# DoHoonKim8/halo2-lasso

Measured on AMD Instinct MI355X. Metric: lasso_prove_time_ms, lower is better.
Workload: dtype u256 (BN254 Fr/Fq, 8x u32 Montgomery); 1 GPU; 2^24 AND Lasso lookup (32-bit operands, 4 chunks of 8+8 bits); lookups_per_proof=16777216, pcs=multilinear KZG (BN254), proof_bytes=64256, parallelism=1 GPU

## Files before the change

### bindings/rust/src/sys.rs

```rust
#![allow(non_camel_case_types, dead_code)]
use halo2_curves::bn256::{Fr, G1Affine, G2Affine};
use std::os::raw::{c_char, c_int, c_void};

pub type lh_status = c_int;
pub const LH_OK: lh_status = 0;
pub const LH_ERR_INVALID_SUMCHECK: lh_status = -1;
pub const LH_ERR_INVALID_PCS_PARAM: lh_status = -2;
pub const LH_ERR_INVALID_PCS_OPEN: lh_status = -3;
pub const LH_ERR_INVALID_SNARK: lh_status = -4;
pub const LH_ERR_SERIALIZATION: lh_status = -5;
pub const LH_ERR_TRANSCRIPT: lh_status = -6;
pub const LH_ERR_DEVICE: lh_status = -7;
pub const LH_ERR_ARG: lh_status = -8;

pub const LH_SC_MAX_TERMS: usize = 48;
pub const LH_SC_MAX_FACTORS: usize = 4;
pub const LH_SC_EVALUATIONS: c_int = 0;
pub const LH_SC_COEFFICIENTS: c_int = 1;
pub const LH_LASSO_MAX_CHUNKS: usize = 8;
pub const LH_LASSO_MAX_MEMORIES: usize = 16;
pub const LH_LASSO_MAX_TERMS: usize = 16;
pub const LH_RCCL_UNIQUE_ID_BYTES: usize = 128;

#[repr(C)] pub struct lh_ctx { _p: [u8; 0] }
// ... 112 lines not shown
    pub preprocess_comms: *const G1Affine,
    pub num_permutation_polys: usize,
    pub permutation_comms: *const G1Affine,
    pub num_lasso_lookups: usize,
    pub lasso_lookups: *const lh_hp_lasso_lookup,
}
#[repr(C)]
pub struct lh_hp_circuit {
    pub user: *mut c_void,
    pub synthesize: Option<unsafe extern "C" fn(*mut c_void, usize, *const Fr, usize, *mut *const c_void, usize) -> c_int>,
}

#[repr(C)]
#[derive(Clone, Copy, Debug, Default)]
pub struct lh_lasso_route {
    pub open_small_depth: u32,
    pub open_small_passes: u32,
    pub eq_factored_rounds: u32,
    pub standard_rounds: u32,
    pub rw_leaf_rounds: u32,
    pub resident_tails: u32,
    pub resident_rounds: u32,
    pub packed_ts_pairs: u32,
    pub derived_commitments: u32,
    pub sorted_dim_reuse: u32,
    pub sharded_rounds: u32,
    pub shard_exchanges: u32,
    pub window_table_jobs: u32,
    pub open_precommit: u32,
    pub resident_layers: u32,
    pub pp_folds: u32,
    pub msm_half_batches: u32,
    pub reserved: [u32; 7],
}

extern "C" {
    pub fn lh_last_error() -> *const c_char;
    pub fn lh_version() -> *const c_char;
    pub fn lh_ctx_create(device_id: c_int, out: *mut *mut lh_ctx) -> lh_status;
    pub fn lh_ctx_destroy(ctx: *mut lh_ctx);
    pub fn lh_ctx_sync(ctx: *mut lh_ctx) -> lh_status;
    pub fn lh_ctx_stream(ctx: *mut lh_ctx) -> *mut c_void;
    pub fn lh_alloc(ctx: *mut lh_ctx, bytes: usize, d_out: *mut *mut c_void) -> lh_status;
    pub fn lh_free(ctx: *mut lh_ctx, d_ptr: *mut c_void) -> lh_status;
    pub fn lh_upload(ctx: *mut lh_ctx, d_dst: *mut c_void, src: *const c_void, bytes: usize) -> lh_status;
    pub fn lh_download(ctx: *mut lh_ctx, dst: *mut c_void, d_src: *const c_void, bytes: usize) -> lh_status;
    pub fn lh_fr_from_u64(ctx: *mut lh_ctx, d_in: *const u64, n: usize, d_out: *mut Fr) -> lh_status;
    pub fn lh_fr_from_u32(ctx: *mut lh_ctx, d_in: *const u32, n: usize, d_out: *mut Fr) -> lh_status;
    pub fn lh_fr_batch_invert(ctx: *mut lh_ctx, d_in: *const Fr, n: usize, d_out: *mut Fr) -> lh_status;
    pub fn lh_fix_var(ctx: *mut lh_ctx, d_in: *const Fr, n_in: usize, x: *const Fr, d_out: *mut Fr) -> lh_status;
    pub fn lh_eq_xy(ctx: *mut lh_ctx, y: *const Fr, num_vars: usize, d_out: *mut Fr) -> lh_status;
    pub fn lh_evaluate(ctx: *mut lh_ctx, d_polys: *const *const Fr, num_polys: usize, num_vars: usize,
                       point: *const Fr, out_evals: *mut Fr) -> lh_status;
    pub fn lh_lincomb(ctx: *mut lh_ctx, d_polys: *const *const Fr, w: *const Fr, num_polys: usize, n: usize,
                      d_out: *mut Fr) -> lh_status;
    pub fn lh_sumcheck_prove(ctx: *mut lh_ctx, prover_kind: c_int, num_vars: usize, expr: *const lh_sop,
                             d_polys: *const *const Fr, num_polys: usize, ys: *const Fr, num_ys: usize,
                             sum: *const Fr, t: *mut lh_transcript, out_challenges: *mut Fr, out_evals: *mut Fr) -> lh_status;
    pub fn lh_sumcheck_prove_expr(ctx: *mut lh_ctx, num_vars: usize, expr: *const lh_expr, d_polys: *const *const Fr,
                                  num_polys: usize, challenges: *const Fr, num_challenges: usize, ys: *const Fr,
                                  num_ys: usize, sum: *const Fr, t: *mut lh_transcript, out_challenges: *mut Fr,
                                  out_evals: *mut Fr) -> lh_status;
    pub fn lh_sumcheck_verify(prover_kind: c_int, num_vars: usize, degree: usize, sum: *const Fr,
                              t: *mut lh_transcript, out_eval: *mut Fr, out_x: *mut Fr) -> lh_status;
    pub fn lh_gkr_fractional_prove(ctx: *mut lh_ctx, num_batching: usize, num_vars: usize,
                                   claimed_p_0s: *const *const Fr, claimed_q_0s: *const *const Fr,
// ... 68 lines not shown
```

### halo2-lasso_amd/__init__.py

```python
import ctypes as C

from . import _ffi
from ._ffi import (lh_fr, lh_g1, lh_sop, lh_evaluation, lh_lasso_table, lh_transcript,
                   LH_SC_EVALUATIONS, LH_SC_COEFFICIENTS)

R_MOD = 0x30644E72E131A029B85045B68181585D2833E84879B9709143E1F593F0000001
Q_MOD = 0x30644E72E131A029B85045B68181585D97816A916871CA8D3C208C16D87CFD47
_MONT = 1 << 256
_MONT_INV_R = pow(_MONT, -1, R_MOD)
_MONT_INV_Q = pow(_MONT, -1, Q_MOD)

SUBTABLE_IDENTITY, SUBTABLE_AND, SUBTABLE_XOR = 0, 1, 2


class Error(Exception):
    code = None


class InvalidSumcheck(Error):
    code = _ffi.LH_ERR_INVALID_SUMCHECK


class InvalidPcsParam(Error):
    code = _ffi.LH_ERR_INVALID_PCS_PARAM
# ... 857 lines not shown
    ctx._comm_keepalive = None


def shard_of(column, rank, size, shard_bit):
    rho = size.bit_length() - 1
    n = len(column)
    return column.reshape(n >> (shard_bit + rho), size, 1 << shard_bit)[:, rank, :].reshape(-1).copy()


def shard_poly(poly, rank, size, shard_bit):
    rho = size.bit_length() - 1
    n_local = (1 << poly.num_vars) >> rho
    out = poly.ctx.alloc(32 * n_local)
    _check(poly.ctx.lib.lh_shard_extract(poly.ctx.h, poly.ptr, n_local, shard_bit, rho, rank, 32, out.ptr))
    return MultilinearPolynomial(poly.ctx, out, poly.num_vars - rho)


def lasso_prove_sharded(pp, table, num_vars, dims_local, transcript):
    if len(dims_local) != table.c:
        raise ArgumentError("expected %d dim columns" % table.c)
    t = table.to_c()
    _check(pp.ctx.lib.lh_lasso_prove_sharded(pp.ctx.h, pp.h, C.byref(t), num_vars, _ptr_array(dims_local), transcript.p))


def lasso_last_timing(ctx):
    out = (C.c_double * _ffi.LH_LASSO_NUM_PHASES)()
    _check(ctx.lib.lh_lasso_last_timing(ctx.h, out))
    names = ["witness", "commit", "surge", "leaves", "gkr", "evals", "open_n", "open_l", "total"]
    return dict(zip(names, list(out)))


ROUTE_FIELDS = ["open_small_depth", "open_small_passes", "eq_factored_rounds", "standard_rounds", "rw_leaf_rounds",
                "resident_tails", "resident_rounds", "packed_ts_pairs", "derived_commitments", "sorted_dim_reuse",
                "sharded_rounds", "shard_exchanges", "window_table_jobs", "open_precommit", "resident_layers", "pp_folds", "msm_half_batches"]


def lasso_last_route(ctx):
    out = (C.c_uint32 * 24)()
    _check(ctx.lib.lh_lasso_last_route(ctx.h, out))
    return dict(zip(ROUTE_FIELDS, [int(v) for v in out]))


def set_option(ctx, name, value):
    _check(ctx.lib.lh_ctx_set_option(ctx.h, name.encode(), int(value)))


def get_option(ctx, name):
    out = C.c_int64(0)
    _check(ctx.lib.lh_ctx_get_option(ctx.h, name.encode(), C.byref(out)))
    return int(out.value)


def profile_enable(ctx, on=True):
    _check(ctx.lib.lh_profile_enable(ctx.h, int(on)))


def profile_read(ctx):
    n = C.c_size_t()
    _check(ctx.lib.lh_profile_read(ctx.h, None, 0, C.byref(n)))
    arr = (_ffi.lh_prof_rec * max(n.value, 1))()
    _check(ctx.lib.lh_profile_read(ctx.h, arr, n.value, C.byref(n)))
    return [dict(name=r.name.decode(), ms=r.ms, bytes=r.bytes, muls=r.muls, items=r.items) for r in arr[:n.value]]


from . import expression
```

### halo2-lasso_amd/csrc/dev.cpp

```cpp
#include <string.h>
#include <stdlib.h>
#include <ctype.h>
#include <sched.h>
#include <atomic>
#include <condition_variable>
#include <mutex>
#include <thread>
#include <functional>
#include <memory>
#include <emmintrin.h>
#include <hip/hip_ext.h>
#include <vector>
#include <chrono>
#include "dev.hpp"

namespace lh {

static thread_local std::string g_last_error;
void set_last_error(const char* msg) { g_last_error = msg ? msg : ""; }
const char* get_last_error() { return g_last_error.c_str(); }

Arena::~Arena() {
  for (auto& b : blocks_) (void)hipFree(b.p);
}
// ... 25 lines not shown
    if (want < bytes) want = bytes;
    void* p = nullptr;
    LH_HIP(hipMalloc(&p, want));
    blocks_.push_back(Block{(char*)p, want, 0});
    cur_ = blocks_.size() - 1;
  }
}

void Arena::release(Mark m) {
  if (blocks_.empty()) return;
  for (size_t i = m.block + 1; i < blocks_.size(); i++) blocks_[i].used = 0;
  cur_ = m.block;
  blocks_[cur_].used = m.used;
}

void Ctx::opt_in_lds(const void* fn, int bytes) {
  for (const void* f : lds_opted)
    if (f == fn) return;
  LH_HIP(hipFuncSetAttribute(fn, hipFuncAttributeMaxDynamicSharedMemorySize, bytes));
  lds_opted.push_back(fn);
}

static const struct {
  const char* name;
  int64_t Options::*field;
  int64_t lo, hi;
} OPTION_TABLE[] = {
    {"open_small_min_vars", &Options::open_small_min_vars, 0, 64}, {"open_small_depth", &Options::open_small_depth, 0, 2},
    {"sc_eq_factoring", &Options::sc_eq_factoring, 0, 1},          {"lasso_pack_ts", &Options::lasso_pack_ts, 0, 1},
    {"sc_tail", &Options::sc_tail, 0, 1},                          {"sc_tail_max_len", &Options::sc_tail_max_len, 0, (int64_t)1 << 20},
    {"shard_exchange_log", &Options::shard_exchange_log, 0, 40},   {"msm_window_tables", &Options::msm_window_tables, 0, 40},
    {"open_precommit", &Options::open_precommit, 0, 64},           {"gkr_resident", &Options::gkr_resident, 0, 1},
    {"sc_pp_fold", &Options::sc_pp_fold, 0, 2},                    {"msm_half_batches", &Options::msm_half_batches, 0, 1},
    {"comm_round", &Options::comm_round, 0, 2},
};

int64_t* Options::find(const char* name) {
  if (!name) return nullptr;
  for (const auto& o : OPTION_TABLE)
    if (strcmp(o.name, name) == 0) return &(this->*o.field);
  return nullptr;
}
bool Options::in_range(const char* name, int64_t value) {
  if (!name) return false;
  for (const auto& o : OPTION_TABLE)
    if (strcmp(o.name, name) == 0) return value >= o.lo && value <= o.hi;
  return false;
}

Options::Options() {
  for (const auto& o : OPTION_TABLE) {
    std::string env = "LH_";
    for (const char* p = o.name; *p; p++) env.push_back((char)toupper((unsigned char)*p));
    const char* e = getenv(env.c_str());
    if (!e || !*e) continue;
    const int64_t v = (int64_t)atoll(e);
    if (v < o.lo || v > o.hi) {
      fprintf(stderr, "[lasso-hip] %s=%s is outside [%lld, %lld]: ignored\n", env.c_str(), e, (long long)o.lo, (long long)o.hi);
      continue;
    }
    this->*o.field = v;
    if (o.field == &Options::open_small_min_vars) open_small_min_vars_forced = true;
  }
}

void Ctx::host_stamp(const char* tag) {
  if (!host_trace_on) return;
// ... 392 lines not shown
```

### halo2-lasso_amd/csrc/dev.hpp

```cpp
#pragma once
#include <hip/hip_runtime_api.h>
#include <stdint.h>
#include <stdarg.h>
#include <stdio.h>
#include <functional>
#include <string>
#include <vector>
#include <utility>
#include <stdexcept>

#include "../../include/lasso_hip.h"
#include "ec.cuh"

namespace lh {

struct Error : std::exception {
  int code;
  std::string msg;
  Error(int c, std::string m) : code(c), msg(std::move(m)) {}
  const char* what() const noexcept override { return msg.c_str(); }
};

void set_last_error(const char* msg);

// ... 50 lines not shown
  char name[40];
  double ms;
  double bytes;
  double muls;
  double items;
};

struct ScFinishArgs {
  uint32_t* ticket;
  uint32_t last_ticket;
  Fr* out_host;
  uint32_t* flag;
  uint32_t seq;
  uint64_t* wide;
  uint32_t tag;
  uint64_t* lanes;
};
constexpr uint32_t FIN_LANE_SUMS = 65536;
constexpr unsigned SC_LANE_TAG_SHIFT = 40;

struct Options {
  int64_t open_small_min_vars = 21;
  bool open_small_min_vars_forced = false;
  int64_t open_small_depth = 0;
  int64_t sc_eq_factoring = 1;
  int64_t lasso_pack_ts = 1;
  int64_t sc_tail = 1;
  int64_t sc_tail_max_len = 8192;
  int64_t shard_exchange_log = 19;
  int64_t open_precommit = 1;
  int64_t msm_window_tables = 0;
  int64_t sc_pp_fold = 1;
  int64_t msm_half_batches = 1;
  int64_t gkr_resident = 1;
  int64_t comm_round = 0;
  Options();
  int64_t* find(const char* name);
  static bool in_range(const char* name, int64_t value);
};
struct RouteStats {
  uint32_t v[LH_LASSO_ROUTE_WORDS] = {0};
  enum { OPEN_DEPTH, OPEN_PASSES, EF_ROUNDS, STD_ROUNDS, RW_ROUNDS, TAILS, TAIL_ROUNDS, PACKED_TS, DERIVED, SORTED_REUSE,
         SHARDED_ROUNDS, SHARD_EXCHANGES, WIN_TABLE_JOBS, OPEN_PRECOMMIT, RESIDENT_LAYERS, PP_FOLDS, MSM_HALF_BATCHES };
};

class HostWorker {
 public:
  HostWorker();
  ~HostWorker();
  void submit(std::function<void()> fn);
  void wait();
 private:
  struct Impl;
  Impl* impl_;
};

struct Ctx {
  Options opt;
  RouteStats route;
  int device = 0;
  hipStream_t stream = nullptr;
  Arena arena;
  void* pinned = nullptr;
  size_t pinned_bytes = 0;
  int num_cus = 256;
  int wall_clock_khz = 100000;
  double lasso_ms[LH_LASSO_NUM_PHASES] = {0};
  lh_comm comm = {0, 1, nullptr, nullptr, nullptr};
  bool has_comm = false;
  bool comm_loopback = false;
  size_t shard_bit = 0;
  bool shard_active = false;
  void* rccl_comm = nullptr;
  void* comm_stage = nullptr;
  size_t comm_stage_bytes = 0;
  uint64_t comm_stats[2] = {0, 0};
// ... 450 lines not shown
```

### halo2-lasso_amd/csrc/msm.hip

```cpp
#include <hip/hip_runtime.h>
#include <algorithm>
#include <exception>
#include <functional>
#include <thread>
#include <vector>
#include <mutex>
#include "dev.hpp"
#include "ff_host.hpp"

namespace lh {

constexpr int MSM_MAX_JOBS = 48;
constexpr uint32_t SENTINEL = 0xffffffffu;
constexpr uint32_t SKIP_IDX = 0x7fffffffu;

struct MsmJobDev {
  const void* scalars;
  const G1Affine* bases;
  uint32_t is_u32;
  uint32_t n;
  uint32_t c, W;
  uint32_t key_base;
  uint32_t entry_base;
  uint32_t win_stride;
  uint32_t is_signed;
  uint32_t seg_base;
  uint32_t seg_per_win;
  uint32_t seg_size;
  uint32_t win_base;
  uint32_t presorted;
  uint32_t pack_shift;
  uint32_t red_W;
  uint32_t nsplit;
  uint32_t share_base;
  uint32_t two_level;
  uint32_t grp_base;
  uint32_t sum_per_win;
  uint32_t merged;
};
constexpr uint32_t KEY_BLOCK_BITS = 10;
// ... 72 lines not shown
        }
      }
      size_t e = (size_t)jb.entry_base + (size_t)w * jb.n + i;
      keys[e] = jb.key_base + (jb.merged ? 0u : w * jb.win_stride) + (jb.pack_shift ? d : (d ? d - 1u : 0u));
      vals[e] = d ? (((uint32_t)i + (jb.merged ? w * jb.n : 0u)) | neg) : SKIP_IDX;
    };
#pragma unroll
    for (int k = 0; k < 8; k++) {
      if (k < nlimbs) {
        buf |= (uint64_t)limb[k] << have;
        have += 32;
        while (have >= (int)c && w < jb.W) {
          emit((uint32_t)buf & mask);
          buf >>= c;
          have -= c;
          w++;
        }
      }
    }
    while (w < jb.W) {
      emit((uint32_t)buf & mask);
      buf >>= c;
      w++;
    }
  }
}


__device__ __forceinline__ const MsmJobDev& job_of_key(const MsmPlanDev& plan, uint32_t key) {
  return plan.job[plan.job_of_block[key >> KEY_BLOCK_BITS]];
}

constexpr int ACC_GROUP = 16;
__global__ __launch_bounds__(128)
void msm_accumulate0_kernel(MsmPlanDev plan, size_t total,
                                                              const uint32_t* __restrict__ sorted_key,
                                                              const uint32_t* __restrict__ sorted_idx, uint32_t K,
                                                              G1Xyzz* __restrict__ buckets,
                                                              uint32_t* __restrict__ cont_key,
                                                              G1Xyzz* __restrict__ cont_pt, size_t nchunks,
                                                              uint32_t* __restrict__ cont_count) {
  __shared__ uint32_t lds_key[ACC_GROUP * 128], lds_idx[ACC_GROUP * 128];
  for (size_t t = (size_t)blockIdx.x * blockDim.x + threadIdx.x; t < nchunks; t += (size_t)gridDim.x * blockDim.x) {
    const size_t p0 = t * K < total ? t * K : total, p1 = p0 + K < total ? p0 + K : total;
    uint32_t ck = SENTINEL;
    if (p0 < p1) {
      uint32_t cur = sorted_key[p0];
      bool cont = p0 > 0 && sorted_key[p0 - 1] == cur;
      const G1Affine* bases = job_of_key(plan, cur).bases;
      G1Xyzz acc = G1Xyzz::identity();
      for (size_t g0 = p0; g0 < p1; g0 += ACC_GROUP) {
        const uint32_t cnt = (uint32_t)(p1 - g0 < (size_t)ACC_GROUP ? p1 - g0 : (size_t)ACC_GROUP);
        for (uint32_t q = 0; q < cnt; q += 4) {
          const uint4 kv = *(const uint4*)(sorted_key + g0 + q), iv4 = *(const uint4*)(sorted_idx + g0 + q);
          lds_key[(q + 0) * 128 + threadIdx.x] = kv.x, lds_key[(q + 1) * 128 + threadIdx.x] = kv.y;
          lds_key[(q + 2) * 128 + threadIdx.x] = kv.z, lds_key[(q + 3) * 128 + threadIdx.x] = kv.w;
          lds_idx[(q + 0) * 128 + threadIdx.x] = iv4.x, lds_idx[(q + 1) * 128 + threadIdx.x] = iv4.y;
          lds_idx[(q + 2) * 128 + threadIdx.x] = iv4.z, lds_idx[(q + 3) * 128 + threadIdx.x] = iv4.w;
        }
        for (uint32_t j = 0; j < cnt; j++) {
          const uint32_t k = lds_key[j * 128 + threadIdx.x];
          if (k != cur) {
            if (cont) {
              ck = cur;
              cont_pt[t] = canon_xyzz(acc);
            } else {
              buckets[cur] = canon_xyzz(acc);
            }
            cont = false;
            acc = G1Xyzz::identity();
            cur = k;
            bases = job_of_key(plan, cur).bases;
          }
          const uint32_t iv = lds_idx[j * 128 + threadIdx.x];
          if (iv != SKIP_IDX) acc = add_mixed_lazy(acc, bases[iv & 0x7fffffffu], (iv >> 31) != 0);
        }
      }
      if (cont) {
        ck = cur;
        cont_pt[t] = canon_xyzz(acc);
      } else {
        buckets[cur] = canon_xyzz(acc);
      }
    }
    cont_key[t] = ck;
    if (ck != SENTINEL) atomicAdd(cont_count, 1u);
  }
}

__global__ __launch_bounds__(128) void msm_accumulate_n_kernel(const uint32_t* __restrict__ in_key,
                                                               const G1Xyzz* __restrict__ in_pt, size_t n_in,
                                                               uint32_t G, G1Xyzz* __restrict__ buckets,
                                                               uint32_t* __restrict__ out_key,
                                                               G1Xyzz* __restrict__ out_pt,
                                                               const uint32_t* __restrict__ in_count,
                                                               uint32_t* __restrict__ out_count) {
  if (*in_count == 0) return;
  for (size_t p = (size_t)blockIdx.x * blockDim.x + threadIdx.x; p < n_in; p += (size_t)gridDim.x * blockDim.x) {
    const uint32_t k = in_key[p];
    const bool valid = k != SENTINEL;
    const bool prev_same = valid && p > 0 && in_key[p - 1] == k;
    const bool slot_owner = (p % G) == 0;
    const bool forced = prev_same && slot_owner;
    uint32_t ok = SENTINEL;
    if (valid && (!prev_same || forced)) {
      G1Xyzz acc = in_pt[p];
      for (size_t q = p + 1; q < n_in && (q % G) != 0 && in_key[q] == k; q++) acc = add(acc, in_pt[q]);
      if (forced) {
        ok = k;
        out_pt[p / G] = acc;
        atomicAdd(out_count, 1u);
      } else {
        buckets[k] = add(buckets[k], acc);
      }
    }
// ... 591 lines not shown
        hipLaunchKernelGGL(msm_presorted_kernel, dim3((unsigned)std::min<size_t>((jd.n + 255) / 256, 4096)), dim3(256), 0,
                           c.stream, jd.key_base, in.sorted_scalars, in.sorted_index, (size_t)jd.n, s.skey + jd.entry_base,
                           s.sidx + jd.entry_base);
        continue;
      }
      if (jd.merged) {
        const size_t e = jd.entry_base;
        sorts.push_back(SortSlab{s.ukey + e, s.skey + e, s.uidx + e, s.sidx + e, (size_t)jd.n * jd.W, s.sort_bits[j]});
        continue;
      }
      for (uint32_t w = 0; w < jd.W; w++) {
        const size_t e = (size_t)jd.entry_base + (size_t)w * jd.n;
        sorts.push_back(SortSlab{s.ukey + e, s.skey + e, s.uidx + e, s.sidx + e, jd.n, s.sort_bits[j]});
      }
    }
    if (!sorts.empty()) sort_pairs_u32_batched(c, sorts.data(), sorts.size());
  }
}

static void msm_sub_accumulate(Ctx& c, MsmSub& s, hipStream_t stream) {
  MsmPlanDev& plan = s.plan;
  {
    ProfScope ps(c, "msm_accumulate0", 96.0 * s.full_pts + 68.0 * (s.total_pts - s.full_pts), 10.0 * (double)s.max_entries, (double)s.max_entries);
    const size_t acc_grid = std::min<size_t>((s.nchunks + 127) / 128, 1 << 16);
    Ctx::LiveRec lr;
    if (c.live) {
      memset(&lr.rec, 0, sizeof(lr.rec));
      snprintf(lr.rec.name, sizeof lr.rec.name, "msm_accumulate0");
      lr.rec.bytes = 96.0 * s.full_pts + 68.0 * (s.total_pts - s.full_pts), lr.rec.muls = 10.0 * (double)s.max_entries;
      lr.rec.items = (double)s.max_entries;
      lr.e0 = c.live_event(), lr.e1 = c.live_event(), lr.batch = c.live_batch;
      LH_HIP(hipEventRecord(lr.e0, stream));
    }
    hipLaunchKernelGGL(msm_accumulate0_kernel, dim3((unsigned)acc_grid), dim3(128), 0, stream, plan, s.max_entries, s.skey, s.sidx,
                       s.K, s.buckets, s.ckey, s.cpt, s.nchunks, s.lvl_cnt);
    if (c.live) {
      LH_HIP(hipEventRecord(lr.e1, stream));
      c.live_recs.push_back(lr);
    }
  }
}

static void msm_sub_tail(Ctx& c, const MsmJob* jobs, MsmSub& s, hipStream_t stream, const ScFinishArgs& fin) {
  const size_t nj = s.idx.size();
  MsmPlanDev& plan = s.plan;
  {
    ProfScope ps(c, "msm_accumulate_levels", 0, 0, (double)s.nchunks);
    msm_continuation_levels(c, stream, s.ckey, s.cpt, s.nchunks, s.buckets, s.lvl_cnt);
  }
  if (s.num_derived) {
    MsmDerivedDev dd;
    memset(&dd, 0, sizeof(dd));
    for (size_t j = 0; j < nj; j++) {
      if (!s.derived[j]) continue;
      const MsmJob& in = jobs[s.idx[j]];
      size_t p = nj;
      for (size_t q = 0; q < nj; q++)
        if ((long)s.idx[q] == (long)in.derived_parent) p = q;
      LH_REQUIRE(p < nj, LH_ERR_ARG, "msm: a derived job lost its parent");
      const uint32_t k = dd.count++;
      dd.off[k + 1] = dd.off[k] + (1u << in.table_in_bits);
      dd.key_base[k] = plan.job[j].key_base;
      dd.parent_key_base[k] = plan.job[p].key_base;
      dd.table[k] = in.d_table, dd.order[k] = in.d_order;
    }
    const size_t nd = dd.off[dd.count];
    ProfScope ps(c, "msm_derived", 132.0 * nd, 14.0 * nd, (double)nd);
    uint32_t* dkey = c.arena.alloc_n<uint32_t>(nd);
// ... 316 lines not shown
```

### include/lasso_hip.h

```cpp
#ifndef LASSO_HIP_H
#define LASSO_HIP_H

#include <stddef.h>
#include <stdint.h>

#ifdef __cplusplus
extern "C" {
#endif

typedef struct { uint64_t l[4]; } lh_fr;
typedef struct { uint64_t x[4], y[4]; } lh_g1;

typedef int lh_status;
#define LH_OK 0
#define LH_ERR_INVALID_SUMCHECK (-1)
#define LH_ERR_INVALID_PCS_PARAM (-2)
#define LH_ERR_INVALID_PCS_OPEN (-3)
#define LH_ERR_INVALID_SNARK (-4)
#define LH_ERR_SERIALIZATION (-5)
#define LH_ERR_TRANSCRIPT (-6)
#define LH_ERR_DEVICE (-7)
#define LH_ERR_ARG (-8)

typedef struct lh_ctx lh_ctx;
// ... 102 lines not shown
lh_status lh_mkzg_open(lh_ctx*, const lh_srs*, const lh_fr* d_poly, size_t num_vars,
                       const lh_fr* point, lh_transcript* t, lh_fr* out_eval);
typedef struct lh_evaluation { uint32_t poly, point; lh_fr value; } lh_evaluation;
lh_status lh_mkzg_batch_open(lh_ctx*, const lh_srs*, size_t num_vars,
                             const lh_fr* const* d_polys, size_t num_polys,
                             const lh_fr* points, size_t num_points,
                             const lh_evaluation* evals, size_t num_evals, lh_transcript* t);

#define LH_SUBTABLE_IDENTITY 0
#define LH_SUBTABLE_AND 1
#define LH_SUBTABLE_XOR 2
#define LH_LASSO_MAX_CHUNKS 8
#define LH_LASSO_MAX_MEMORIES 16
#define LH_LASSO_MAX_TERMS 16
typedef struct lh_lasso_table {
  uint32_t num_chunks;
  uint32_t chunk_bits;
  uint32_t num_memories;
  uint32_t memory_chunk[LH_LASSO_MAX_MEMORIES];
  uint32_t memory_subtable[LH_LASSO_MAX_MEMORIES];
  uint32_t num_terms;
  lh_fr g_coeff[LH_LASSO_MAX_TERMS];
  uint8_t g_num_factors[LH_LASSO_MAX_TERMS];
  uint8_t g_factor[LH_LASSO_MAX_TERMS][LH_SC_MAX_FACTORS];
} lh_lasso_table;
lh_status lh_lasso_prove(lh_ctx*, const lh_srs*, const lh_lasso_table*, size_t num_vars,
                         const uint32_t* const* d_dims, lh_transcript* t);

#define LH_LASSO_NUM_PHASES 9
lh_status lh_lasso_last_timing(lh_ctx*, double* out_ms);

lh_status lh_ctx_set_option(lh_ctx*, const char* name, int64_t value);
lh_status lh_ctx_get_option(lh_ctx*, const char* name, int64_t* out);
#define LH_LASSO_ROUTE_WORDS 24
typedef struct lh_lasso_route {
  uint32_t open_small_depth;
  uint32_t open_small_passes;
  uint32_t eq_factored_rounds;
  uint32_t standard_rounds;
  uint32_t rw_leaf_rounds;
  uint32_t resident_tails;
  uint32_t resident_rounds;
  uint32_t packed_ts_pairs;
  uint32_t derived_commitments;
  uint32_t sorted_dim_reuse;
  uint32_t sharded_rounds;
  uint32_t shard_exchanges;
  uint32_t window_table_jobs;
  uint32_t open_precommit;
  uint32_t resident_layers;
  uint32_t pp_folds;
  uint32_t msm_half_batches;
  uint32_t reserved[7];
} lh_lasso_route;
lh_status lh_lasso_last_route(lh_ctx*, lh_lasso_route* out);

typedef struct lh_comm {
  int rank, size;
  void* user;
  int (*all_gather)(void* user, const void* send, void* recv, size_t bytes_per_rank);
  int (*all_gather_device)(void* user, const void* d_send, void* d_recv, size_t bytes_per_rank, void* hip_stream);
} lh_comm;
lh_status lh_ctx_set_comm(lh_ctx*, const lh_comm* comm, size_t shard_bit);
#define LH_RCCL_UNIQUE_ID_BYTES 128
lh_status lh_rccl_unique_id(uint8_t out[LH_RCCL_UNIQUE_ID_BYTES]);
lh_status lh_ctx_set_comm_rccl(lh_ctx*, int rank, int size, const uint8_t unique_id[LH_RCCL_UNIQUE_ID_BYTES],
                               size_t shard_bit);
lh_status lh_ctx_set_comm_loopback(lh_ctx*, int rank, int size, size_t shard_bit);
lh_status lh_ctx_comm_stats(lh_ctx*, uint64_t out[2]);
lh_status lh_ctx_comm_phase_stats(lh_ctx*, uint64_t out[16], int reset);
lh_status lh_ctx_memory_stats(lh_ctx*, uint64_t out[4]);
lh_status lh_ctx_host_cpus(lh_ctx*, char* bus_id, size_t bus_id_cap, char* cpulist, size_t cpulist_cap);
lh_status lh_lasso_prove_sharded(lh_ctx*, const lh_srs*, const lh_lasso_table*, size_t num_vars,
                                 const uint32_t* const* d_dims_local, lh_transcript* t);

typedef struct lh_hp_lookup {
  const lh_expr* inputs;
  const lh_expr* tables;
  size_t width;
} lh_hp_lookup;
#define LH_HP_LASSO_MAX_COMMITMENTS 63
typedef struct lh_hp_lasso_lookup {
  lh_lasso_table table;
  size_t output_poly;
  size_t chunk_polys[LH_LASSO_MAX_CHUNKS];
} lh_hp_lasso_lookup;
// ... 132 lines not shown
```

Measured before the change: 55.24 ms.

## Accumulate MSM buckets in 9x29-bit lazy-reduction limbs for cheaper field multiplies

Adds a 29-bit-limb Montgomery field representation with column-wise 64-bit accumulation, plus a mixed XYZZ point addition built on it. The first MSM bucket-accumulation kernel is templated and uses this representation by default, converting to and from the 32-bit form at the boundaries. The aim is to cut the carry-propagation cost of 256-bit modular multiplies in the hottest MSM loop, at the price of conversion overhead, higher register pressure, and more complex edge-case handling for the doubling and identity cases.

```diff
diff --git a/bindings/rust/src/sys.rs b/bindings/rust/src/sys.rs
--- a/bindings/rust/src/sys.rs
+++ b/bindings/rust/src/sys.rs
@@ -168,6 +168,7 @@
     pub pp_folds: u32,
     pub msm_half_batches: u32,
     pub reserved: [u32; 7],
+    pub msm29_batches: u32,
 }
 
 extern "C" {
diff --git a/halo2-lasso_amd/__init__.py b/halo2-lasso_amd/__init__.py
--- a/halo2-lasso_amd/__init__.py
+++ b/halo2-lasso_amd/__init__.py
@@ -913,13 +913,14 @@
 
 ROUTE_FIELDS = ["open_small_depth", "open_small_passes", "eq_factored_rounds", "standard_rounds", "rw_leaf_rounds",
                 "resident_tails", "resident_rounds", "packed_ts_pairs", "derived_commitments", "sorted_dim_reuse",
-                "sharded_rounds", "shard_exchanges", "window_table_jobs", "open_precommit", "resident_layers", "pp_folds", "msm_half_batches"]
+                "sharded_rounds", "shard_exchanges", "window_table_jobs", "open_precommit", "resident_layers", "pp_folds", "msm_half_batches",
+                None, None, None, None, None, None, None, "msm29_batches"]
 
 
 def lasso_last_route(ctx):
-    out = (C.c_uint32 * 24)()
+    out = (C.c_uint32 * len(ROUTE_FIELDS))()
     _check(ctx.lib.lh_lasso_last_route(ctx.h, out))
-    return dict(zip(ROUTE_FIELDS, [int(v) for v in out]))
+    return {k: int(v) for k, v in zip(ROUTE_FIELDS, out) if k}
 
 
 def set_option(ctx, name, value):
diff --git a/halo2-lasso_amd/csrc/dev.cpp b/halo2-lasso_amd/csrc/dev.cpp
--- a/halo2-lasso_amd/csrc/dev.cpp
+++ b/halo2-lasso_amd/csrc/dev.cpp
@@ -81,7 +81,7 @@
     {"shard_exchange_log", &Options::shard_exchange_log, 0, 40},   {"msm_window_tables", &Options::msm_window_tables, 0, 40},
     {"open_precommit", &Options::open_precommit, 0, 64},           {"gkr_resident", &Options::gkr_resident, 0, 1},
     {"sc_pp_fold", &Options::sc_pp_fold, 0, 2},                    {"msm_half_batches", &Options::msm_half_batches, 0, 1},
-    {"comm_round", &Options::comm_round, 0, 2},
+    {"comm_round", &Options::comm_round, 0, 2},                    {"msm_limbs29", &Options::msm_limbs29, 0, 1},
 };
 
 int64_t* Options::find(const char* name) {
diff --git a/halo2-lasso_amd/csrc/dev.hpp b/halo2-lasso_amd/csrc/dev.hpp
--- a/halo2-lasso_amd/csrc/dev.hpp
+++ b/halo2-lasso_amd/csrc/dev.hpp
@@ -106,6 +106,7 @@
   int64_t msm_window_tables = 0;
   int64_t sc_pp_fold = 1;
   int64_t msm_half_batches = 1;
+  int64_t msm_limbs29 = 1;
   int64_t gkr_resident = 1;
   int64_t comm_round = 0;
   Options();
@@ -115,7 +116,8 @@
 struct RouteStats {
   uint32_t v[LH_LASSO_ROUTE_WORDS] = {0};
   enum { OPEN_DEPTH, OPEN_PASSES, EF_ROUNDS, STD_ROUNDS, RW_ROUNDS, TAILS, TAIL_ROUNDS, PACKED_TS, DERIVED, SORTED_REUSE,
-         SHARDED_ROUNDS, SHARD_EXCHANGES, WIN_TABLE_JOBS, OPEN_PRECOMMIT, RESIDENT_LAYERS, PP_FOLDS, MSM_HALF_BATCHES };
+         SHARDED_ROUNDS, SHARD_EXCHANGES, WIN_TABLE_JOBS, OPEN_PRECOMMIT, RESIDENT_LAYERS, PP_FOLDS, MSM_HALF_BATCHES,
+         RESERVED0, RESERVED1, RESERVED2, RESERVED3, RESERVED4, RESERVED5, RESERVED6, MSM29_BATCHES };
 };
 
 class HostWorker {
diff --git a/halo2-lasso_amd/csrc/ec29.cuh b/halo2-lasso_amd/csrc/ec29.cuh
--- /dev/null
+++ b/halo2-lasso_amd/csrc/ec29.cuh
@@ -0,0 +1,98 @@
+#pragma once
+#include "ec.cuh"
+#include "ff29.cuh"
+
+namespace lh {
+
+struct G1Xyzz29 {
+  Fq29 x, y, zz, zzz;
+};
+
+LH_HD bool is_zero_limbs29(const Fq29& a) {
+  uint32_t o = 0;
+#pragma unroll
+  for (int i = 0; i < 9; i++) o |= a.l[i];
+  return o == 0;
+}
+template <int N>
+LH_HD bool is_zero_mod29(const Fq29& a) {
+  bool cand = false;
+#pragma unroll
+  for (int k = 0; k < N; k++) cand = cand || a.l[0] == kmod29v<FqParams>(k, 0);
+  if (!cand) return false;
+  bool z = false;
+#pragma unroll
+  for (int k = 0; k < N; k++) {
+    bool e = true;
+#pragma unroll
+    for (int i = 0; i < 9; i++) e = e && a.l[i] == kmod29v<FqParams>(k, i);
+    z = z || e;
+  }
+  return z;
+}
+
+LH_HD Fq29 to29(const Fq& x) {
+  Fq v = x;
+#pragma unroll
+  for (int k = 0; k < 5; k++) v = add(v, v);
+  return slice29(v);
+}
+LH_HD G1Xyzz29 identity29() {
+  G1Xyzz29 r;
+#pragma unroll
+  for (int i = 0; i < 9; i++) r.x.l[i] = r.y.l[i] = r.zz.l[i] = r.zzz.l[i] = 0;
+  return r;
+}
+LH_HD G1Xyzz to_xyzz(const G1Xyzz29& p) {
+  G1Xyzz r;
+  r.x = div32_29(p.x), r.y = div32_29(p.y), r.zz = div32_29(p.zz), r.zzz = div32_29(p.zzz);
+  return r;
+}
+LH_HD G1Xyzz29 from_xyzz(const G1Xyzz& p) {
+  G1Xyzz29 r;
+  r.x = to29(p.x), r.y = to29(p.y), r.zz = to29(p.zz), r.zzz = to29(p.zzz);
+  return r;
+}
+
+LH_HD G1Xyzz29 add_mixed29(const G1Xyzz29& p, const G1Affine& q, bool negate) {
+  typedef FqParams P;
+  if (q.is_identity()) return p;
+  const Fq29 qx = slice29_x32(q.x);
+  Fq29 qy = slice29_x32(q.y);
+  if (negate) {
+    Fq29 z;
+#pragma unroll
+    for (int i = 0; i < 9; i++) z.l[i] = 0;
+    qy = sub29<P, 32>(z, qy);
+  }
+  if (is_zero_limbs29(p.zz)) {
+    G1Xyzz29 r;
+    r.x = qx, r.y = qy;
+    r.zz = r.zzz = one29<P>();
+    return r;
+  }
+  const Fq29 u2 = mul29(qx, p.zz), s2 = mul29(qy, p.zzz);
+  const Fq29 pp_ = sub29<P, 32>(u2, p.x), r_ = sub29<P, 32>(s2, p.y);
+  const Fq29 pp = mul29(pp_, pp_);
+  const Fq29 zz3 = mul29(p.zz, pp);
+  if (is_zero_mod29<2>(zz3)) {
+    if (!is_zero_mod29<8>(mul29(r_, r_))) return identity29();
+    G1Affine qa;
+    qa.x = div32_29(qx), qa.y = div32_29(qy);
+    return from_xyzz(dbl_affine(qa));
+  }
+  const Fq29 ppp = mul29(pp_, pp), qq = mul29(p.x, pp), rr = mul29(r_, r_);
+  G1Xyzz29 r;
+  r.x = sub29<P, 5>(sub29<P, 3>(rr, ppp), add29(qq, qq));
+  {
+    Fq29 z;
+#pragma unroll
+    for (int i = 0; i < 9; i++) z.l[i] = 0;
+    r.y = dot29(r_, sub29<P, 16>(qq, r.x), sub29<P, 32>(z, p.y), ppp);
+  }
+  r.zz = zz3;
+  r.zzz = mul29(p.zzz, ppp);
+  return r;
+}
+
+}
diff --git a/halo2-lasso_amd/csrc/ff29.cuh b/halo2-lasso_amd/csrc/ff29.cuh
--- /dev/null
+++ b/halo2-lasso_amd/csrc/ff29.cuh
@@ -0,0 +1,312 @@
+#pragma once
+#include "ff.cuh"
+
+namespace lh {
+
+constexpr uint32_t M29 = (1u << 29) - 1u;
+
+template <class P>
+struct Fp29 {
+  uint32_t l[9];
+};
+
+template <class P>
+LH_HD constexpr uint32_t mod29(int i) {
+  const int bit = 29 * i, w = bit >> 5, s = bit & 31;
+  uint64_t v = w < 8 ? (uint64_t)P::mod(w) >> s : 0;
+  if (s && w + 1 < 8) v |= (uint64_t)P::mod(w + 1) << (32 - s);
+  return (uint32_t)v & M29;
+}
+template <class P>
+LH_HD constexpr uint32_t kmod29v(int k, int i);
+template <class P, int K>
+LH_HD constexpr uint32_t kmod29(int i) {
+  return kmod29v<P>(K, i);
+}
+template <class P>
+LH_HD constexpr uint32_t kmod29v(int k, int i) {
+  uint64_t carry = 0, limb = 0;
+  for (int j = 0; j <= i; j++) {
+    const uint64_t v = (uint64_t)k * mod29<P>(j) + carry;
+    limb = j < 8 ? (v & M29) : v;
+    carry = v >> 29;
+  }
+  return (uint32_t)limb;
+}
+template <class P>
+LH_HD constexpr uint32_t ninv29() {
+  const uint32_t n0 = P::mod(0);
+  uint32_t inv = 1;
+  for (int it = 0; it < 6; it++) inv *= 2u - n0 * inv;
+  return (0u - inv) & M29;
+}
+
+#if defined(__HIP_DEVICE_COMPILE__)
+#define LH_MAD29(x, y) (acc += (uint64_t)(x) * (y))
+#define LH_MAD29S(x, sc) (acc += (uint64_t)(x) * (sc))
+#define LH_MAD29_2(x0, y0, x1, y1) (LH_MAD29(x0, y0), LH_MAD29(x1, y1))
+#define LH_MAD29_3(x0, y0, x1, y1, x2, y2) (LH_MAD29(x0, y0), LH_MAD29(x1, y1), LH_MAD29(x2, y2))
+template <int LO, int HI, int K>
+__device__ __forceinline__ void mad29_run(uint64_t& acc, const uint32_t* x, const uint32_t* y) {
+  if constexpr (HI - LO + 1 >= 3) {
+    LH_MAD29_3(x[LO], y[K - LO], x[LO + 1], y[K - LO - 1], x[LO + 2], y[K - LO - 2]);
+    mad29_run<LO + 3, HI, K>(acc, x, y);
+  } else if constexpr (HI - LO + 1 == 2) {
+    LH_MAD29_2(x[LO], y[K - LO], x[LO + 1], y[K - LO - 1]);
+  } else if constexpr (HI - LO + 1 == 1) {
+    LH_MAD29(x[LO], y[K - LO]);
+  }
+}
+#define LH_MAD29S_2(x0, s0, x1, s1) (LH_MAD29(x0, s0), LH_MAD29(x1, s1))
+#define LH_MAD29S_3(x0, s0, x1, s1, x2, s2) (LH_MAD29(x0, s0), LH_MAD29(x1, s1), LH_MAD29(x2, s2))
+template <class P, int LO, int HI, int K>
+__device__ __forceinline__ void mad29_run_mod(uint64_t& acc, const uint32_t* m) {
+  if constexpr (HI - LO + 1 >= 3) {
+    LH_MAD29S_3(m[LO], mod29<P>(K - LO), m[LO + 1], mod29<P>(K - LO - 1), m[LO + 2], mod29<P>(K - LO - 2));
+    mad29_run_mod<P, LO + 3, HI, K>(acc, m);
+  } else if constexpr (HI - LO + 1 == 2) {
+    LH_MAD29S_2(m[LO], mod29<P>(K - LO), m[LO + 1], mod29<P>(K - LO - 1));
+  } else if constexpr (HI - LO + 1 == 1) {
+    LH_MAD29S(m[LO], mod29<P>(K - LO));
+  }
+}
+template <class P, int K>
+__device__ __forceinline__ void mul29_column(uint64_t& acc, const uint32_t* a, const uint32_t* b, uint32_t* m, uint32_t* r) {
+  constexpr int LO = K < 9 ? 0 : K - 8, HI = K < 9 ? K : 8;
+  mad29_run<LO, HI, K>(acc, a, b);
+  if constexpr (K < 9) {
+    if constexpr (K >= 1) mad29_run_mod<P, 0, K - 1, K>(acc, m);
+    m[K] = ((uint32_t)acc * ninv29<P>()) & M29;
+    LH_MAD29S(m[K], mod29<P>(0));
+  } else {
+    mad29_run_mod<P, LO, 8, K>(acc, m);
+    r[K - 9] = (uint32_t)acc & M29;
+  }
+  acc >>= 29;
+  if constexpr (K < 16) mul29_column<P, K + 1>(acc, a, b, m, r);
+}
+template <class P>
+__device__ __forceinline__ Fp29<P> mul29(const Fp29<P>& a, const Fp29<P>& b) {
+  uint64_t acc = 0;
+  uint32_t m[9];
+  Fp29<P> r;
+  mul29_column<P, 0>(acc, a.l, b.l, m, r.l);
+  r.l[8] = (uint32_t)acc;
+  return r;
+}
+template <class P, int K>
+__device__ __forceinline__ void dot29_column(uint64_t& acc, const uint32_t* a0, const uint32_t* b0, const uint32_t* a1,
+                                             const uint32_t* b1, uint32_t* m, uint32_t* r) {
+  constexpr int LO = K < 9 ? 0 : K - 8, HI = K < 9 ? K : 8;
+  mad29_run<LO, HI, K>(acc, a0, b0);
+  mad29_run<LO, HI, K>(acc, a1, b1);
+  if constexpr (K < 9) {
+    if constexpr (K >= 1) mad29_run_mod<P, 0, K - 1, K>(acc, m);
+    m[K] = ((uint32_t)acc * ninv29<P>()) & M29;
+    LH_MAD29S(m[K], mod29<P>(0));
+  } else {
+    mad29_run_mod<P, LO, 8, K>(acc, m);
+    r[K - 9] = (uint32_t)acc & M29;
+  }
+  acc >>= 29;
+  if constexpr (K < 16) dot29_column<P, K + 1>(acc, a0, b0, a1, b1, m, r);
+}
+template <class P>
+__device__ __forceinline__ Fp29<P> dot29(const Fp29<P>& a0, const Fp29<P>& b0, const Fp29<P>& a1, const Fp29<P>& b1) {
+  uint64_t acc = 0;
+  uint32_t m[9];
+  Fp29<P> r;
+  dot29_column<P, 0>(acc, a0.l, b0.l, a1.l, b1.l, m, r.l);
+  r.l[8] = (uint32_t)acc;
+  return r;
+}
+#undef LH_MAD29
+#undef LH_MAD29S
+#undef LH_MAD29_2
+#undef LH_MAD29_3
+#undef LH_MAD29S_2
+#undef LH_MAD29S_3
+#else
+template <class P>
+LH_HD Fp29<P> mul29(const Fp29<P>& a, const Fp29<P>& b) {
+  uint64_t acc = 0;
+  uint32_t m[9];
+  Fp29<P> r;
+  for (int k = 0; k < 17; k++) {
+    for (int i = (k < 9 ? 0 : k - 8); i <= (k < 9 ? k : 8); i++) acc += (uint64_t)a.l[i] * b.l[k - i];
+    for (int i = (k < 9 ? 0 : k - 8); i <= (k < 9 ? k - 1 : 8); i++) acc += (uint64_t)m[i] * mod29<P>(k - i);
+    if (k < 9) {
+      m[k] = ((uint32_t)acc * ninv29<P>()) & M29;
+      acc += (uint64_t)m[k] * mod29<P>(0);
+    } else {
+      r.l[k - 9] = (uint32_t)acc & M29;
+    }
+    acc >>= 29;
+  }
+  r.l[8] = (uint32_t)acc;
+  return r;
+}
+template <class P>
+LH_HD Fp29<P> dot29(const Fp29<P>& a0, const Fp29<P>& b0, const Fp29<P>& a1, const Fp29<P>& b1) {
+  uint64_t acc = 0;
+  uint32_t m[9];
+  Fp29<P> r;
+  for (int k = 0; k < 17; k++) {
+    for (int i = (k < 9 ? 0 : k - 8); i <= (k < 9 ? k : 8); i++) acc += (uint64_t)a0.l[i] * b0.l[k - i] + (uint64_t)a1.l[i] * b1.l[k - i];
+    for (int i = (k < 9 ? 0 : k - 8); i <= (k < 9 ? k - 1 : 8); i++) acc += (uint64_t)m[i] * mod29<P>(k - i);
+    if (k < 9) {
+      m[k] = ((uint32_t)acc * ninv29<P>()) & M29;
+      acc += (uint64_t)m[k] * mod29<P>(0);
+    } else {
+      r.l[k - 9] = (uint32_t)acc & M29;
+    }
+    acc >>= 29;
+  }
+  r.l[8] = (uint32_t)acc;
+  return r;
+}
+#endif
+
+template <class P>
+LH_HD Fp29<P> carry29(const int32_t* t) {
+  Fp29<P> r;
+  int32_t c = 0;
+#pragma unroll
+  for (int i = 0; i < 8; i++) {
+    const int32_t v = t[i] + c;
+    r.l[i] = (uint32_t)v & M29;
+    c = v >> 29;
+  }
+  r.l[8] = (uint32_t)(t[8] + c);
+  return r;
+}
+template <class P>
+LH_HD Fp29<P> add29(const Fp29<P>& a, const Fp29<P>& b) {
+  int32_t t[9];
+#pragma unroll
+  for (int i = 0; i < 9; i++) t[i] = (int32_t)(a.l[i] + b.l[i]);
+  return carry29<P>(t);
+}
+template <class P, int K>
+LH_HD Fp29<P> sub29(const Fp29<P>& a, const Fp29<P>& b) {
+  int32_t t[9];
+#pragma unroll
+  for (int i = 0; i < 9; i++) {
+    t[i] = (int32_t)(a.l[i] + kmod29<P, K>(i)) - (int32_t)b.l[i];
+  }
+  return carry29<P>(t);
+}
+
+template <class P>
+LH_HD Fp29<P> slice29(const Fp<P>& x) {
+  Fp29<P> r;
+#pragma unroll
+  for (int i = 0; i < 9; i++) {
+    const int bit = 29 * i, w = bit >> 5, s = bit & 31;
+    uint64_t v = w < 8 ? (uint64_t)x.l[w] >> s : 0;
+    if (s && w + 1 < 8) v |= (uint64_t)x.l[w + 1] << (32 - s);
+    r.l[i] = (uint32_t)v & M29;
+  }
+  return r;
+}
+template <class P>
+LH_HD Fp<P> unslice29(const Fp29<P>& x) {
+  Fp<P> r;
+#pragma unroll
+  for (int w = 0; w < 8; w++) {
+    uint64_t v = 0;
+#pragma unroll
+    for (int i = 0; i < 9; i++) {
+      const int shift = 29 * i - 32 * w;
+      if (shift > -29 && shift < 32) v |= shift >= 0 ? (uint64_t)x.l[i] << shift : (uint64_t)x.l[i] >> (-shift);
+    }
+    r.l[w] = (uint32_t)v;
+  }
+  return r;
+}
+
+template <class P>
+LH_HD constexpr uint32_t one29(int i) {
+  uint32_t v[8] = {};
+  for (int j = 0; j < 8; j++) v[j] = P::r1(j);
+  for (int d = 0; d < 5; d++) {
+    uint32_t top = 0;
+    for (int j = 0; j < 8; j++) {
+      const uint32_t n = (v[j] << 1) | top;
+      top = v[j] >> 31;
+      v[j] = n;
+    }
+    bool ge = true;
+    for (int j = 7; j >= 0; j--)
+      if (v[j] != P::mod(j)) {
+        ge = v[j] > P::mod(j);
+        break;
+      }
+    if (ge) {
+      uint64_t b = 0;
+      for (int j = 0; j < 8; j++) {
+        const uint64_t t = (uint64_t)v[j] - P::mod(j) - b;
+        v[j] = (uint32_t)t;
+        b = (t >> 32) & 1u;
+      }
+    }
+  }
+  const int bit = 29 * i, w = bit >> 5, s = bit & 31;
+  uint64_t x = w < 8 ? (uint64_t)v[w] >> s : 0;
+  if (s && w + 1 < 8) x |= (uint64_t)v[w + 1] << (32 - s);
+  return (uint32_t)x & M29;
+}
+template <class P>
+LH_HD Fp29<P> one29() {
+  Fp29<P> r;
+#pragma unroll
+  for (int i = 0; i < 9; i++) r.l[i] = one29<P>(i);
+  return r;
+}
+
+template <class P>
+LH_HD Fp29<P> slice29_x32(const Fp<P>& x) {
+  Fp29<P> r;
+  r.l[0] = (x.l[0] << 5) & M29;
+#pragma unroll
+  for (int i = 1; i < 9; i++) {
+    const int bit = 29 * i - 5, w = bit >> 5, s = bit & 31;
+    uint64_t v = (uint64_t)x.l[w] >> s;
+    if (s && w + 1 < 8) v |= (uint64_t)x.l[w + 1] << (32 - s);
+    r.l[i] = (uint32_t)v & M29;
+  }
+  return r;
+}
+template <class P>
+LH_HD Fp<P> div32_29(const Fp29<P>& v) {
+  uint32_t u[9];
+#pragma unroll
+  for (int w = 0; w < 9; w++) {
+    uint32_t x = 0;
+#pragma unroll
+    for (int i = 0; i < 9; i++) {
+      const int shift = 29 * i - 32 * w;
+      if (shift > -29 && shift < 32) x |= shift >= 0 ? v.l[i] << shift : v.l[i] >> (-shift);
+    }
+    u[w] = x;
+  }
+  const uint32_t k = (u[0] * (ninv29<P>() & 31u)) & 31u;
+  uint32_t t[9];
+  uint64_t c = 0;
+#pragma unroll
+  for (int j = 0; j < 8; j++) {
+    c += (uint64_t)k * P::mod(j) + u[j];
+    t[j] = (uint32_t)c;
+    c >>= 32;
+  }
+  t[8] = u[8] + (uint32_t)c;
+  Fp<P> r;
+#pragma unroll
+  for (int j = 0; j < 8; j++) r.l[j] = (t[j] >> 5) | (t[j + 1] << 27);
+  return reduce_once(r);
+}
+
+using Fq29 = Fp29<FqParams>;
+using Fr29 = Fp29<FrParams>;
+
+}
diff --git a/halo2-lasso_amd/csrc/msm.hip b/halo2-lasso_amd/csrc/msm.hip
--- a/halo2-lasso_amd/csrc/msm.hip
+++ b/halo2-lasso_amd/csrc/msm.hip
@@ -6,6 +6,7 @@
 #include <vector>
 #include <mutex>
 #include "dev.hpp"
+#include "ec29.cuh"
 #include "ff_host.hpp"
 
 namespace lh {
@@ -144,6 +145,19 @@
 }
 
 constexpr int ACC_GROUP = 16;
+struct Acc32 {
+  typedef G1Xyzz acc_t;
+  static __device__ __forceinline__ acc_t identity() { return G1Xyzz::identity(); }
+  static __device__ __forceinline__ acc_t add(const acc_t& a, const G1Affine& b, bool neg) { return add_mixed_lazy(a, b, neg); }
+  static __device__ __forceinline__ G1Xyzz out(const acc_t& a) { return canon_xyzz(a); }
+};
+struct Acc29 {
+  typedef G1Xyzz29 acc_t;
+  static __device__ __forceinline__ acc_t identity() { return identity29(); }
+  static __device__ __forceinline__ acc_t add(const acc_t& a, const G1Affine& b, bool neg) { return add_mixed29(a, b, neg); }
+  static __device__ __forceinline__ G1Xyzz out(const acc_t& a) { return to_xyzz(a); }
+};
+template <class A>
 __global__ __launch_bounds__(128)
 void msm_accumulate0_kernel(MsmPlanDev plan, size_t total,
                                                               const uint32_t* __restrict__ sorted_key,
@@ -160,7 +174,7 @@
       uint32_t cur = sorted_key[p0];
       bool cont = p0 > 0 && sorted_key[p0 - 1] == cur;
       const G1Affine* bases = job_of_key(plan, cur).bases;
-      G1Xyzz acc = G1Xyzz::identity();
+      typename A::acc_t acc = A::identity();
       for (size_t g0 = p0; g0 < p1; g0 += ACC_GROUP) {
         const uint32_t cnt = (uint32_t)(p1 - g0 < (size_t)ACC_GROUP ? p1 - g0 : (size_t)ACC_GROUP);
         for (uint32_t q = 0; q < cnt; q += 4) {
@@ -175,24 +189,24 @@
           if (k != cur) {
             if (cont) {
               ck = cur;
-              cont_pt[t] = canon_xyzz(acc);
+              cont_pt[t] = A::out(acc);
             } else {
-              buckets[cur] = canon_xyzz(acc);
+              buckets[cur] = A::out(acc);
             }
             cont = false;
-            acc = G1Xyzz::identity();
+            acc = A::identity();
             cur = k;
             bases = job_of_key(plan, cur).bases;
           }
           const uint32_t iv = lds_idx[j * 128 + threadIdx.x];
-          if (iv != SKIP_IDX) acc = add_mixed_lazy(acc, bases[iv & 0x7fffffffu], (iv >> 31) != 0);
+          if (iv != SKIP_IDX) acc = A::add(acc, bases[iv & 0x7fffffffu], (iv >> 31) != 0);
         }
       }
       if (cont) {
         ck = cur;
-        cont_pt[t] = canon_xyzz(acc);
+        cont_pt[t] = A::out(acc);
       } else {
-        buckets[cur] = canon_xyzz(acc);
+        buckets[cur] = A::out(acc);
       }
     }
     cont_key[t] = ck;
@@ -850,8 +864,14 @@
       lr.e0 = c.live_event(), lr.e1 = c.live_event(), lr.batch = c.live_batch;
       LH_HIP(hipEventRecord(lr.e0, stream));
     }
-    hipLaunchKernelGGL(msm_accumulate0_kernel, dim3((unsigned)acc_grid), dim3(128), 0, stream, plan, s.max_entries, s.skey, s.sidx,
-                       s.K, s.buckets, s.ckey, s.cpt, s.nchunks, s.lvl_cnt);
+    if (c.opt.msm_limbs29) {
+      c.route.v[RouteStats::MSM29_BATCHES]++;
+      hipLaunchKernelGGL(msm_accumulate0_kernel<Acc29>, dim3((unsigned)acc_grid), dim3(128), 0, stream, plan, s.max_entries, s.skey,
+                         s.sidx, s.K, s.buckets, s.ckey, s.cpt, s.nchunks, s.lvl_cnt);
+    } else {
+      hipLaunchKernelGGL(msm_accumulate0_kernel<Acc32>, dim3((unsigned)acc_grid), dim3(128), 0, stream, plan, s.max_entries, s.skey,
+                         s.sidx, s.K, s.buckets, s.ckey, s.cpt, s.nchunks, s.lvl_cnt);
+    }
     if (c.live) {
       LH_HIP(hipEventRecord(lr.e1, stream));
       c.live_recs.push_back(lr);
diff --git a/include/lasso_hip.h b/include/lasso_hip.h
--- a/include/lasso_hip.h
+++ b/include/lasso_hip.h
@@ -158,7 +158,7 @@
 
 lh_status lh_ctx_set_option(lh_ctx*, const char* name, int64_t value);
 lh_status lh_ctx_get_option(lh_ctx*, const char* name, int64_t* out);
-#define LH_LASSO_ROUTE_WORDS 24
+#define LH_LASSO_ROUTE_WORDS 25
 typedef struct lh_lasso_route {
   uint32_t open_small_depth;
   uint32_t open_small_passes;
@@ -178,6 +178,7 @@
   uint32_t pp_folds;
   uint32_t msm_half_batches;
   uint32_t reserved[7];
+  uint32_t msm29_batches;
 } lh_lasso_route;
 lh_status lh_lasso_last_route(lh_ctx*, lh_lasso_route* out);
 
```

Result: no change. 54.89 ms, median of 6 (-0.6%).
